# cloneofsimo/lora

Measured on AMD Instinct MI355X. Metric: train steps/sec SD1.5 rank-4 512^2 (train_lora_dreambooth.py step), higher is better.
Workload: dtype bf16

## Files before the change

### include/lora_amd.h

```cpp
#ifndef LORA_AMD_H
#define LORA_AMD_H

#include <stddef.h>
#include <stdint.h>

#ifdef __cplusplus
extern "C" {
#endif

#define LORA_AMD_ABI_VERSION 7

#define LORA_AMD_OK 0
#define LORA_AMD_EINVAL (-1)
#define LORA_AMD_ERANK (-2)
#define LORA_AMD_ELAUNCH (-3)
#define LORA_AMD_EWORKSPACE (-4)
#define LORA_AMD_EUNSUPPORTED (-5)

#define LORA_AMD_MAX_RANK 64

#define LORA_AMD_F32 0
#define LORA_AMD_F16 1
#define LORA_AMD_BF16 2

// ... 445 lines not shown
                                  int32_t r, int32_t act_dtype, float scale, float dropout_p, uint64_t seed, uint64_t offset,
                                  const uint64_t *offset_dev, void *stream);
int lora_amd_sum_parts(const float *part, int32_t nparts, int64_t stride, float *out, int64_t n, void *stream);


size_t lora_amd_sumsq_workspace(int64_t n);
int lora_amd_sumsq(const float *g, int64_t n, float *out_sumsq, void *workspace,
                   size_t workspace_bytes, void *stream);

typedef struct lora_amd_adamw_group {
  int64_t begin, end;
  float lr;
  float weight_decay;
} lora_amd_adamw_group;

int lora_amd_clip_adamw(float *p, float *g, float *exp_avg, float *exp_avg_sq,
                        int64_t n, const lora_amd_adamw_group *groups_dev,
                        int32_t n_groups, const float *sumsq, float grad_scale,
                        float max_norm, float beta1, float beta2, float eps,
                        int64_t step, int32_t zero_grad, void *stream);

int lora_amd_clip_adamw_dev(float *p, float *g, float *exp_avg, float *exp_avg_sq,
                            int64_t n, const lora_amd_adamw_group *groups_dev,
                            int32_t n_groups, const float *sumsq, float grad_scale,
                            float max_norm, float beta1, float beta2, float eps,
                            const int64_t *step_dev, const float *scaler, int32_t zero_grad, void *stream);
int lora_amd_step_advance(int64_t *step_dev, void *stream);

int lora_amd_loss_scale_update(float *state, const float *sumsq, int64_t *step_dev, float growth_factor,
                               float backoff_factor, int32_t growth_interval, void *stream);

int lora_amd_ti_rows_step(void *table, const void *table_grad, const int64_t *ids_dev, int32_t n_tokens,
                          int32_t hidden, int32_t table_dtype, float *rows, float *exp_avg, float *exp_avg_sq,
                          float lr, float beta1, float beta2, float eps, float weight_decay, float grad_scale,
                          int64_t step, float decay_lambda, float target_norm, void *stream);


size_t lora_amd_groupnorm_workspace(int32_t B, int32_t C, int32_t HW, int32_t groups);
int lora_amd_groupnorm_supported(int32_t B, int32_t C, int32_t HW, int32_t groups);
int lora_amd_groupnorm_fwd(const void *x, const void *gamma, const void *beta, void *y, float *stats,
                           void *workspace, size_t workspace_bytes, int32_t B, int32_t C, int32_t HW,
                           int32_t groups, float eps, int32_t act, int32_t dtype, void *stream);
int lora_amd_groupnorm_bwd(const void *x, const void *gout, const void *gamma, const void *beta,
                           const float *stats, void *dx, void *workspace, size_t workspace_bytes, int32_t B,
                           int32_t C, int32_t HW, int32_t groups, int32_t act, int32_t dtype, void *stream);

size_t lora_amd_groupnorm_nhwc_workspace(int32_t B, int32_t C, int32_t HW, int32_t groups);
int lora_amd_groupnorm_nhwc_fwd(const void *x, const void *gamma, const void *beta, const float *addend, void *y,
                                float *aff, void *workspace, size_t workspace_bytes, int32_t B, int32_t C, int32_t HW,
                                int32_t groups, float eps, int32_t act, int32_t dtype, void *stream);
int lora_amd_groupnorm_nhwc_bwd(const void *x, const void *gout, const void *gamma, const float *aff, void *dx,
                                void *workspace, size_t workspace_bytes, int32_t B, int32_t C, int32_t HW,
                                int32_t groups, int32_t act, int32_t dtype, void *stream);

int lora_amd_layernorm_supported(int32_t K);
int lora_amd_layernorm_fwd(const void *x, const void *gamma, const void *beta, void *y, float *stats, int64_t M,
                           int32_t K, float eps, int32_t dtype, void *stream);
int lora_amd_layernorm_bwd(const void *x, const void *gout, const void *gamma, const float *stats, void *dx,
                           int64_t M, int32_t K, int32_t dtype, void *stream);
int lora_amd_add_layernorm_fwd(const void *x, const void *res, const void *gamma, const void *beta, void *sum_out,
                               void *y, float *stats, int64_t M, int32_t K, float eps, int32_t dtype, void *stream);
int lora_amd_add_layernorm_bwd(const void *x, const void *gout, const void *gsum, const void *gamma,
                               const float *stats, void *dx, int64_t M, int32_t K, int32_t dtype, void *stream);

int lora_amd_geglu_fwd(const void *y, int64_t ldy, void *out, int64_t ldo, int64_t M, int32_t inner, int32_t dtype,
                       void *stream);
int lora_amd_geglu_bwd(const void *y, int64_t ldy, const void *gout, int64_t ldg, void *gy, int64_t ldgy, int64_t M,
                       int32_t inner, int32_t dtype, void *stream);

#ifdef __cplusplus
}
#endif
#endif
```

### lora_amd/_C.py

```python
from __future__ import annotations

import ctypes as C
import os
from typing import Dict, Optional, Sequence, Tuple

import torch

_HERE = os.path.dirname(os.path.abspath(__file__))
LIB_PATH = os.path.join(_HERE, "csrc", "liblora_amd.so")

OK = 0
F32, F16, BF16 = 0, 1, 2
FACTOR_RK, FACTOR_KR = 0, 1
ROUND_REFERENCE, ROUND_ONCE, ROUND_DITHER = 0, 1, 2
MAX_RANK = 64
ABI_VERSION = 7

_DT = {torch.float32: F32, torch.float16: F16, torch.bfloat16: BF16}

SYMBOLS = (
    "lora_amd_abi_version", "lora_amd_last_error", "lora_amd_target_arch",
    "lora_amd_merge_plan", "lora_amd_merge_batched", "lora_amd_merge_set_tuning", "lora_amd_merge_step_set_tuning", "lora_amd_rank16_mfma", "lora_amd_factors_mfma_set_tuning",
    "lora_amd_merge_step_plan", "lora_amd_merge_step",
    "lora_amd_rowdot", "lora_amd_rowdot_masked", "lora_amd_rank_update",
    "lora_amd_colreduce_workspace", "lora_amd_colreduce",
    "lora_amd_rowdot_batched", "lora_amd_colreduce_batched", "lora_amd_chol_inverse_batched",
    "lora_amd_ragged_plan", "lora_amd_rowdot_ragged", "lora_amd_colreduce_ragged", "lora_amd_sub_ragged",
    "lora_amd_rowdot16_planes_plan", "lora_amd_rowdot16_planes", "lora_amd_rowdot16_planes_packed", "lora_amd_thin_pack",
    "lora_amd_split16_ragged", "lora_amd_split16_transpose",
    "lora_amd_split16_residual", "lora_amd_thin_gram", "lora_amd_thin_apply", "lora_amd_thin_rotate", "lora_amd_thin_select", "lora_amd_thin_clamp",
    "lora_amd_linear_plan", "lora_amd_linear_fwd", "lora_amd_linear_bwd_g", "lora_amd_linear_bwd_x",
    "lora_amd_linear_bwd_factors", "lora_amd_linear_bwd_factors_drop", "lora_amd_linear_bwd_factors_heads",
    "lora_amd_linear_factors_self_plan", "lora_amd_linear_factors_self_plan_rows", "lora_amd_linear_bwd_factors_self",
    "lora_amd_linear_factors_self_ragged_plan", "lora_amd_linear_bwd_factors_self_ragged",
    "lora_amd_factors_mfma_plan", "lora_amd_factor_pack_plan", "lora_amd_factor_pack",
    "lora_amd_factors_mfma_ragged_plan", "lora_amd_linear_bwd_factors_mfma_ragged", "lora_amd_factors_mfma_block_map",
    "lora_amd_linear_bwd_factors_mfma_ragged_mapped",
    "lora_amd_linear_gemm_fwd_heads",
    "lora_amd_reduce_batched", "lora_amd_linear_gemm_supported", "lora_amd_linear_gemm_fwd",
    "lora_amd_ws_config", "lora_amd_ws_packed_elems", "lora_amd_ws_pack", "lora_amd_linear_ws", "lora_amd_linear_ws_heads",
    "lora_amd_conv_plan", "lora_amd_conv_down_fwd", "lora_amd_conv_up_fwd", "lora_amd_conv_bwd_g", "lora_amd_conv_bwd_x",
    "lora_amd_conv3_nhwc_plan", "lora_amd_conv3_nhwc_pack", "lora_amd_conv3_nhwc_down_fwd", "lora_amd_conv3_nhwc_bwd_dx",
    "lora_amd_conv3_nhwc_bwd_down", "lora_amd_sum_parts",
    "lora_amd_conv3_nhwc_pack_plan", "lora_amd_conv3_nhwc_pack_batched", "lora_amd_conv3_nhwc_fwd_fused",
    "lora_amd_linear_bwd_g_blocks", "lora_amd_linear_bwd_g_folded",
    "lora_amd_sumsq_workspace", "lora_amd_sumsq", "lora_amd_clip_adamw", "lora_amd_clip_adamw_dev",
    "lora_amd_step_advance", "lora_amd_loss_scale_update", "lora_amd_ti_rows_step",
    "lora_amd_groupnorm_workspace", "lora_amd_groupnorm_supported", "lora_amd_groupnorm_fwd", "lora_amd_groupnorm_bwd",
    "lora_amd_geglu_fwd", "lora_amd_geglu_bwd",
    "lora_amd_layernorm_supported", "lora_amd_layernorm_fwd", "lora_amd_layernorm_bwd",
    "lora_amd_groupnorm_nhwc_workspace", "lora_amd_groupnorm_nhwc_fwd", "lora_amd_groupnorm_nhwc_bwd",
    "lora_amd_add_layernorm_fwd", "lora_amd_add_layernorm_bwd",
    "lora_amd_linear_gemm_fwd_rowscale", "lora_amd_rank_update_rowscale", "lora_amd_conv_up_fwd_rowscale",
)


class HipExtensionMissing(RuntimeError):
    pass


class FactorsSelfPlan(C.Structure):
    _fields_ = [("supported", C.c_int32), ("rank_tile", C.c_int32), ("nparts", C.c_int32), ("reserved", C.c_int32),
                ("up_part_floats", C.c_int64), ("down_part_floats", C.c_int64)]


class SelfSite(C.Structure):
    _fields_ = [
        ("g", C.c_void_p), ("x", C.c_void_p), ("down", C.c_void_p), ("up", C.c_void_p),
        ("up_part", C.c_void_p), ("down_part", C.c_void_p),
        ("ldg", C.c_int64), ("ldx", C.c_int64), ("M", C.c_int64),
        ("N", C.c_int32), ("K", C.c_int32), ("r", C.c_int32), ("scale", C.c_float),
        ("g_head_dim", C.c_int32), ("g_head_pad", C.c_int32), ("x_head_dim", C.c_int32), ("x_head_pad", C.c_int32),
        ("rows_per_block", C.c_int32), ("nsplit", C.c_int32), ("kt_g", C.c_int32), ("logL_g", C.c_int32),
        ("kt_x", C.c_int32), ("logL_x", C.c_int32), ("tile_g", C.c_int32), ("nct_g", C.c_int32),
        ("tile_x", C.c_int32), ("nct_x", C.c_int32),
        ("reserved0", C.c_int32), ("reserved", C.c_int32),
        ("block_begin", C.c_int64),
    ]


class FactorsMfmaPlan(C.Structure):
    _fields_ = [("supported", C.c_int32), ("lds_class", C.c_int32), ("rank_tile", C.c_int32),
                ("rows_per_block", C.c_int32), ("nparts", C.c_int32), ("lds_bytes", C.c_int32),
                ("blocks_per_wg", C.c_int32), ("reserved", C.c_int32),
                ("up_part_floats", C.c_int64), ("down_part_floats", C.c_int64),
                ("pack_up_elems", C.c_int64), ("pack_down_elems", C.c_int64)]


class PackSite(C.Structure):
    _fields_ = [("down", C.c_void_p), ("up", C.c_void_p), ("pk_down", C.c_void_p), ("pk_up", C.c_void_p),
                ("N", C.c_int32), ("K", C.c_int32), ("r", C.c_int32), ("reserved", C.c_int32), ("begin", C.c_int64)]


class FmSite(C.Structure):
    _fields_ = [
        ("g", C.c_void_p), ("x", C.c_void_p), ("pk_up", C.c_void_p), ("pk_down", C.c_void_p),
        ("up_part", C.c_void_p), ("down_part", C.c_void_p),
        ("ldg", C.c_int64), ("ldx", C.c_int64), ("M", C.c_int64),
        ("N", C.c_int32), ("K", C.c_int32), ("r", C.c_int32), ("scale", C.c_float),
        ("g_head_dim", C.c_int32), ("g_head_pad", C.c_int32), ("x_head_dim", C.c_int32), ("x_head_pad", C.c_int32),
        ("rows_per_block", C.c_int32), ("blocks_per_wg", C.c_int32),
        ("resident_is_x", C.c_int32), ("cw", C.c_int32), ("nchunk", C.c_int32), ("x_head_magic", C.c_int32),
        ("g_head_magic", C.c_int32), ("lds_bytes", C.c_int32),
        ("block_begin", C.c_int64),
# ... 1912 lines not shown
    _check(require().lora_amd_layernorm_bwd(x.data_ptr(), gout.data_ptr(), gamma.data_ptr(), stats.data_ptr(),
                                            dx.data_ptr(), x.numel() // K, K, dtype_code(x.dtype), _stream()),
           "lora_amd_layernorm_bwd")
    return dx


_gn_nhwc_ws_cache: Dict[Tuple[int, int, int, int], int] = {}


def groupnorm_nhwc_workspace(B: int, C_: int, HW: int, groups: int) -> int:
    key = (B, C_, HW, groups)
    n = _gn_nhwc_ws_cache.get(key)
    if n is None:
        n = _gn_nhwc_ws_cache[key] = int(require().lora_amd_groupnorm_nhwc_workspace(B, C_, HW, groups))
    return n


def groupnorm_nhwc_fwd(x: torch.Tensor, gamma: torch.Tensor, beta: torch.Tensor, groups: int, eps: float,
                       act: bool, addend: Optional[torch.Tensor] = None) -> Tuple[torch.Tensor, torch.Tensor]:
    _dev_check(x, gamma, beta, addend)
    if addend is not None and (addend.dtype != torch.float32 or not addend.is_contiguous()
                               or tuple(addend.shape) != (x.shape[0], x.shape[1])):
        raise ValueError("groupnorm_nhwc_fwd: addend must be a contiguous float32 [B, C] tensor")
    B, C_ = x.shape[0], x.shape[1]
    HW = x.numel() // (B * C_)
    nbytes = groupnorm_nhwc_workspace(B, C_, HW, groups)
    if nbytes == 0:
        raise ValueError(f"lora_amd_groupnorm_nhwc: geometry {tuple(x.shape)} / {groups} groups not supported")
    y = torch.empty_like(x)
    aff = torch.empty(B, 4, C_, dtype=torch.float32, device=x.device)
    ws = torch.empty(nbytes // 4, dtype=torch.float32, device=x.device)
    _check(require().lora_amd_groupnorm_nhwc_fwd(x.data_ptr(), gamma.data_ptr(), beta.data_ptr(), _ptr(addend),
                                                 y.data_ptr(), aff.data_ptr(), ws.data_ptr(), nbytes, B, C_, HW, groups, eps,
                                                 1 if act else 0, dtype_code(x.dtype), _stream()),
           "lora_amd_groupnorm_nhwc_fwd")
    return y, aff


def groupnorm_nhwc_bwd(x: torch.Tensor, gout: torch.Tensor, gamma: torch.Tensor, aff: torch.Tensor, groups: int,
                       act: bool) -> torch.Tensor:
    _dev_check(x, gout, gamma, aff)
    B, C_ = x.shape[0], x.shape[1]
    HW = x.numel() // (B * C_)
    nbytes = groupnorm_nhwc_workspace(B, C_, HW, groups)
    dx = torch.empty_like(x)
    ws = torch.empty(nbytes // 4, dtype=torch.float32, device=x.device)
    _check(require().lora_amd_groupnorm_nhwc_bwd(x.data_ptr(), gout.data_ptr(), gamma.data_ptr(), aff.data_ptr(),
                                                 dx.data_ptr(), ws.data_ptr(), nbytes, B, C_, HW, groups,
                                                 1 if act else 0, dtype_code(x.dtype), _stream()),
           "lora_amd_groupnorm_nhwc_bwd")
    return dx


def add_layernorm_fwd(x: torch.Tensor, res: torch.Tensor, gamma: torch.Tensor, beta: torch.Tensor,
                      eps: float) -> Tuple[torch.Tensor, torch.Tensor, torch.Tensor]:
    _dev_check(x, res, gamma, beta)
    K = x.shape[-1]
    M = x.numel() // K
    s, y = torch.empty_like(x), torch.empty_like(x)
    stats = torch.empty(M, 2, dtype=torch.float32, device=x.device)
    _check(require().lora_amd_add_layernorm_fwd(x.data_ptr(), res.data_ptr(), gamma.data_ptr(), beta.data_ptr(),
                                                s.data_ptr(), y.data_ptr(), stats.data_ptr(), M, K, eps,
                                                dtype_code(x.dtype), _stream()), "lora_amd_add_layernorm_fwd")
    return s, y, stats


def add_layernorm_bwd(s: torch.Tensor, gout: torch.Tensor, gsum: Optional[torch.Tensor], gamma: torch.Tensor,
                      stats: torch.Tensor) -> torch.Tensor:
    _dev_check(s, gout, gsum, gamma, stats)
    K = s.shape[-1]
    dx = torch.empty_like(s)
    _check(require().lora_amd_add_layernorm_bwd(s.data_ptr(), gout.data_ptr(), _ptr(gsum), gamma.data_ptr(),
                                                stats.data_ptr(), dx.data_ptr(), s.numel() // K, K,
                                                dtype_code(s.dtype), _stream()), "lora_amd_add_layernorm_bwd")
    return dx
```

### lora_amd/csrc/hostops.hip

```cpp
#include <algorithm>

#include "common.hpp"

namespace lora_amd {

constexpr int kHT = 256;
constexpr int kHU = 4;
constexpr int kHMaxSlices = 256;

__device__ inline float fast_rcp(float v) { return __builtin_amdgcn_rcpf(v); }
__device__ inline float sigmoidf(float z) { return fast_rcp(1.f + __expf(-z)); }
__device__ inline float silu_grad(float z) {
  const float s = sigmoidf(z);
  return s * (1.f + z * (1.f - s));
}
__device__ inline float erf_as(float x) {
  const float ax = fabsf(x);
  const float t = fast_rcp(1.f + 0.3275911f * ax);
  float p = 1.061405429f;
  p = fmaf(p, t, -1.453152027f);
  p = fmaf(p, t, 1.421413741f);
  p = fmaf(p, t, -0.284496736f);
  p = fmaf(p, t, 0.254829592f);
  const float e = 1.f - p * t * __expf(-ax * ax);
// ... 474 lines not shown
  const float c1 = group_allsum(s1, logL) * inv_n, c2 = group_allsum(s2, logL) * inv_n;
  if (!live) return;
#pragma unroll
  for (int u = 0; u < kLU; ++u) {
    const int cc = l + u * L;
    if (cc < c8) {
      float o[8];
#pragma unroll
      for (int e = 0; e < 8; ++e) o[e] = rstd * (t[u][e] - c1 - xh[u][e] * c2);
      if (ADDG) {
        float gs[8];
        unpack8_sel<E>(gsr[u], true, gs);
#pragma unroll
        for (int e = 0; e < 8; ++e) o[e] += gs[e];
      }
      store8<E>(dx + row * (int64_t)c8 * 8 + cc * 8, o);
    }
  }
}

static inline int ln_logL(int c8) {
  for (int lg = 0; lg <= 6; ++lg)
    if (((c8 + (1 << lg) - 1) >> lg) <= kLU) return lg;
  return -1;
}

constexpr int kNU = 4;

struct GnNhwcGeo {
  int c8, cw, tiles, nslots, px, S;
  bool ok;
};
static GnNhwcGeo gn_nhwc_geo(int B, int C, int HW, int G) {
  GnNhwcGeo q{};
  q.ok = B > 0 && C > 0 && HW > 0 && G > 0 && C % G == 0 && C % 8 == 0;
  if (!q.ok) return q;
  q.c8 = C / 8;
  int best = 1, best_act = 0;
  for (int d = 1; d <= std::min(q.c8, 128); ++d) {
    if (q.c8 % d) continue;
    const int act = (kHT / d) * d;
    if (act >= best_act) { best_act = act; best = d; }
  }
  q.cw = best;
  q.tiles = q.c8 / q.cw;
  q.nslots = kHT / q.cw;
  int64_t px = std::max<int64_t>(2 * q.nslots, (int64_t)HW * B * q.tiles / 768);
  px = std::min<int64_t>(px, HW);
  q.px = (int)px;
  q.S = (HW + q.px - 1) / q.px;
  return q;
}

struct NhwcBlock {
  int b, s, col, slot, np;
  bool active;
  int64_t base;
};
__device__ inline NhwcBlock nhwc_block(int C, int HW, int cw, int tiles, int nslots, int px, int S) {
  NhwcBlock k;
  const int bs = blockIdx.x / tiles, tile = blockIdx.x - bs * tiles;
  k.b = bs / S;
  k.s = bs - k.b * S;
  k.slot = threadIdx.x / cw;
  const int cl = threadIdx.x - k.slot * cw;
  k.active = k.slot < nslots;
  k.col = tile * cw + cl;
  const int p0 = k.s * px;
  k.np = min(px, HW - p0);
  k.base = ((int64_t)k.b * HW + p0) * C + (int64_t)k.col * 8;
  return k;
}

__device__ inline void ld8f(const float *p, float (&v)[8]) {
  typedef float f4 __attribute__((ext_vector_type(4)));
  const f4 a = *reinterpret_cast<const f4 *>(p), b = *reinterpret_cast<const f4 *>(p + 4);
#pragma unroll
  for (int i = 0; i < 4; ++i) { v[i] = a[i]; v[i + 4] = b[i]; }
}
__device__ inline void st8f(float *p, const float (&v)[8]) {
  typedef float f4 __attribute__((ext_vector_type(4)));
  f4 a, b;
#pragma unroll
  for (int i = 0; i < 4; ++i) { a[i] = v[i]; b[i] = v[i + 4]; }
  *reinterpret_cast<f4 *>(p) = a;
  *reinterpret_cast<f4 *>(p + 4) = b;
}

__device__ inline void nhwc_slot_reduce(float (&a0)[8], float (&a1)[8], const NhwcBlock &k, int cw, int nslots,
                                        float *s_red ) {
  if (k.active) {
    st8f(s_red + (size_t)threadIdx.x * 8, a0);
    st8f(s_red + (size_t)(kHT + threadIdx.x) * 8, a1);
  }
  __syncthreads();
  if (k.active && k.slot == 0) {
    for (int sl = 1; sl < nslots; ++sl) {
      float t0[8], t1[8];
      ld8f(s_red + (size_t)(sl * cw + threadIdx.x) * 8, t0);
      ld8f(s_red + (size_t)(kHT + sl * cw + threadIdx.x) * 8, t1);
#pragma unroll
      for (int e = 0; e < 8; ++e) { a0[e] += t0[e]; a1[e] += t1[e]; }
    }
  }
}

// ... 172 lines not shown
      }
      LORA_AMD_LOADS_ISSUED();
#pragma unroll
      for (int u = 0; u < kNU; ++u) {
        const int pp = p + u * nslots;
        if (pp < k.np) {
          float v[8], go[8], t[8], xh[8];
          unpack8_sel<E>(xr[u], true, v);
          unpack8_sel<E>(gr[u], true, go);
          gn_nhwc_terms<E, ACT>(v, go, ga, be, mean, rstd, gam, t, xh);
          if (APPLY) {
            float o[8];
#pragma unroll
            for (int e = 0; e < 8; ++e) o[e] = rstd[e] * (t[e] - c1[e] - xh[e] * c2[e]);
            store8<E>(dx + k.base + (int64_t)pp * C, o);
          } else {
#pragma unroll
            for (int e = 0; e < 8; ++e) {
              s1[e] += t[e];
              s2[e] = fmaf(t[e], xh[e], s2[e]);
            }
          }
        }
      }
    }
  }
  if (!APPLY) {
    nhwc_slot_reduce(s1, s2, k, cw, nslots, s_red);
    if (k.active && k.slot == 0) {
      float *o = part + ((int64_t)(k.b * S + k.s) * 2) * C + (int64_t)k.col * 8;
      st8f(o, s1);
      st8f(o + C, s2);
    }
  }
}

__global__ __launch_bounds__(kHT) void gn_nhwc_bwd_finalize_kernel(const float *__restrict__ part,
                                                                   float *__restrict__ cvec, int C, int HW, int G,
                                                                   int S) {
  __shared__ float s_red[4][2];
  const int b = blockIdx.x / G, g = blockIdx.x - b * G, cpg = C / G;
  float s1 = 0.f, s2 = 0.f;
  for (int i = threadIdx.x; i < S * cpg; i += kHT) {
    const int s = i / cpg, c = g * cpg + (i - s * cpg);
    const float *pp = part + ((int64_t)(b * S + s) * 2) * C + c;
    s1 += pp[0];
    s2 += pp[C];
  }
  block_sum2(s1, s2, s_red);
  const float inv_n = 1.f / ((float)HW * (float)cpg);
  for (int cc = threadIdx.x; cc < cpg; cc += kHT) {
    cvec[(int64_t)b * 2 * C + g * cpg + cc] = s1 * inv_n;
    cvec[(int64_t)b * 2 * C + C + g * cpg + cc] = s2 * inv_n;
  }
}

static inline bool aligned_for(const void *p, int dt) { return ((uintptr_t)p % (dt == LORA_AMD_F32 ? 32 : 16)) == 0; }

}

using namespace lora_amd;

extern "C" size_t lora_amd_groupnorm_workspace(int32_t B, int32_t C, int32_t HW, int32_t groups) {
  const GnGeo q = gn_geo(B, C, HW, groups);
  return q.ok ? (size_t)B * groups * q.S * 2 * sizeof(float) : 0;
}

extern "C" int lora_amd_groupnorm_supported(int32_t B, int32_t C, int32_t HW, int32_t groups) {
  return gn_geo(B, C, HW, groups).ok ? 1 : 0;
}

#define GN_CHECKS(name)                                                                                              \
  const GnGeo q = gn_geo(B, C, HW, groups);                                                                          \
  LORA_AMD_CHECK(q.ok, LORA_AMD_EINVAL, name ": geometry B=%d C=%d HW=%d groups=%d not supported", B, C, HW, groups); \
  LORA_AMD_CHECK(dtype_ok(dtype), LORA_AMD_EINVAL, name ": bad dtype %d", dtype);                                    \
  LORA_AMD_CHECK(workspace_bytes >= lora_amd_groupnorm_workspace(B, C, HW, groups), LORA_AMD_EWORKSPACE,             \
                 name ": workspace %zu < %zu bytes", workspace_bytes, lora_amd_groupnorm_workspace(B, C, HW, groups)); \
  const dim3 grid((unsigned)((int64_t)B * groups * q.S)), block(kHT);                                                \
  hipStream_t st = (hipStream_t)stream;                                                                              \
  float *part = reinterpret_cast<float *>(workspace)

extern "C" int lora_amd_groupnorm_fwd(const void *x, const void *gamma, const void *beta, void *y, float *stats,
                                      void *workspace, size_t workspace_bytes, int32_t B, int32_t C, int32_t HW,
                                      int32_t groups, float eps, int32_t act, int32_t dtype, void *stream) {
  GN_CHECKS("groupnorm_fwd");
  LORA_AMD_CHECK(x && gamma && beta && y && stats && workspace, LORA_AMD_EINVAL, "groupnorm_fwd: null pointer");
  LORA_AMD_CHECK(aligned_for(x, dtype) && aligned_for(y, dtype), LORA_AMD_EINVAL, "groupnorm_fwd: unaligned tensor");
  by_dtype(dtype, [&](auto e) {
    using E = decltype(e);
    using S = typename E::storage;
    hipLaunchKernelGGL((gn_stats_kernel<E>), grid, block, 0, st, (const S *)x, part, groups, q.cpg, HW, q.chunks,
                       q.per_block, q.S);
    by_bool(act != 0, [&](auto a) {
      hipLaunchKernelGGL((gn_apply_kernel<E, decltype(a)::value>), grid, block, 0, st, (const S *)x, (const S *)gamma,
                         (const S *)beta, (S *)y, part, stats, groups, q.cpg, HW, q.chunks, q.per_block, q.S, eps);
    });
  });
  return check_launch("lora_amd_groupnorm_fwd");
}

extern "C" int lora_amd_groupnorm_bwd(const void *x, const void *gout, const void *gamma, const void *beta,
                                      const float *stats, void *dx, void *workspace, size_t workspace_bytes,
                                      int32_t B, int32_t C, int32_t HW, int32_t groups, int32_t act, int32_t dtype,
                                      void *stream) {
  GN_CHECKS("groupnorm_bwd");
  LORA_AMD_CHECK(x && gout && gamma && beta && stats && dx && workspace, LORA_AMD_EINVAL,
// ... 77 lines not shown
}

extern "C" int lora_amd_add_layernorm_fwd(const void *x, const void *res, const void *gamma, const void *beta,
                                          void *sum_out, void *y, float *stats, int64_t M, int32_t K, float eps,
                                          int32_t dtype, void *stream) {
  LN_CHECKS("layernorm_fwd");
  LORA_AMD_CHECK(x && gamma && beta && y && stats, LORA_AMD_EINVAL, "layernorm_fwd: null pointer");
  LORA_AMD_CHECK((res == nullptr) == (sum_out == nullptr), LORA_AMD_EINVAL,
                 "layernorm_fwd: res and sum_out go together");
  LORA_AMD_CHECK(aligned_for(x, dtype) && aligned_for(y, dtype) && aligned_for(gamma, dtype) && aligned_for(beta, dtype) &&
                     aligned_for(res, dtype) && aligned_for(sum_out, dtype),
                 LORA_AMD_EINVAL, "layernorm_fwd: unaligned tensor");
  const bool add = res != nullptr;
  by_dtype(dtype, [&](auto e) {
    by_bool(add, [&](auto a) {
      using S = typename decltype(e)::storage;
      hipLaunchKernelGGL((ln_fwd_kernel<decltype(e), decltype(a)::value>), grid, block, 0, st, (const S *)x, (const S *)res,
                         (const S *)gamma, (const S *)beta, (S *)sum_out, (S *)y, stats, M, c8, logL, eps);
    });
  });
  return check_launch("lora_amd_layernorm_fwd");
}

extern "C" int lora_amd_layernorm_bwd(const void *x, const void *gout, const void *gamma, const float *stats,
                                      void *dx, int64_t M, int32_t K, int32_t dtype, void *stream) {
  return lora_amd_add_layernorm_bwd(x, gout, nullptr, gamma, stats, dx, M, K, dtype, stream);
}

extern "C" int lora_amd_add_layernorm_bwd(const void *x, const void *gout, const void *gsum, const void *gamma,
                                          const float *stats, void *dx, int64_t M, int32_t K, int32_t dtype,
                                          void *stream) {
  LN_CHECKS("layernorm_bwd");
  LORA_AMD_CHECK(x && gout && gamma && stats && dx, LORA_AMD_EINVAL, "layernorm_bwd: null pointer");
  LORA_AMD_CHECK(aligned_for(x, dtype) && aligned_for(gout, dtype) && aligned_for(dx, dtype) && aligned_for(gamma, dtype) &&
                     aligned_for(gsum, dtype),
                 LORA_AMD_EINVAL, "layernorm_bwd: unaligned tensor");
  by_dtype(dtype, [&](auto e) {
    by_bool(gsum != nullptr, [&](auto a) {
      using S = typename decltype(e)::storage;
      hipLaunchKernelGGL((ln_bwd_kernel<decltype(e), decltype(a)::value>), grid, block, 0, st, (const S *)x, (const S *)gout,
                         (const S *)gsum, (const S *)gamma, stats, (S *)dx, M, c8, logL);
    });
  });
  return check_launch("lora_amd_layernorm_bwd");
}

static size_t gn_nhwc_part_floats(const GnNhwcGeo &q, int B, int C) { return (size_t)B * q.S * 2 * C; }

extern "C" size_t lora_amd_groupnorm_nhwc_workspace(int32_t B, int32_t C, int32_t HW, int32_t groups) {
  const GnNhwcGeo q = gn_nhwc_geo(B, C, HW, groups);
  return q.ok ? (gn_nhwc_part_floats(q, B, C) + (size_t)B * 2 * C) * sizeof(float) : 0;
}

#define GN_NHWC_CHECKS(name)                                                                                          \
  const GnNhwcGeo q = gn_nhwc_geo(B, C, HW, groups);                                                                  \
  LORA_AMD_CHECK(q.ok, LORA_AMD_EINVAL, name ": geometry B=%d C=%d HW=%d groups=%d not supported", B, C, HW, groups); \
  LORA_AMD_CHECK(dtype_ok(dtype), LORA_AMD_EINVAL, name ": bad dtype %d", dtype);                                     \
  LORA_AMD_CHECK(workspace_bytes >= lora_amd_groupnorm_nhwc_workspace(B, C, HW, groups), LORA_AMD_EWORKSPACE,         \
                 name ": workspace %zu bytes too small", workspace_bytes);                                            \
  const dim3 grid((unsigned)((int64_t)B * q.S * q.tiles)), gridg((unsigned)(B * groups)), block(kHT);                 \
  hipStream_t st = (hipStream_t)stream;                                                                               \
  float *part = reinterpret_cast<float *>(workspace);                                                                 \
  float *cvec = part + gn_nhwc_part_floats(q, B, C);                                                                  \
  (void)cvec

extern "C" int lora_amd_groupnorm_nhwc_fwd(const void *x, const void *gamma, const void *beta, const float *addend,
                                           void *y, float *aff, void *workspace, size_t workspace_bytes, int32_t B, int32_t C, int32_t HW,
                                           int32_t groups, float eps, int32_t act, int32_t dtype, void *stream) {
  GN_NHWC_CHECKS("groupnorm_nhwc_fwd");
  LORA_AMD_CHECK(x && gamma && beta && y && aff && workspace, LORA_AMD_EINVAL, "groupnorm_nhwc_fwd: null pointer");
  LORA_AMD_CHECK(aligned_for(x, dtype) && aligned_for(y, dtype) && ((uintptr_t)aff % 32) == 0, LORA_AMD_EINVAL,
                 "groupnorm_nhwc_fwd: unaligned tensor");
  by_dtype(dtype, [&](auto e) {
    using E = decltype(e);
    using S = typename E::storage;
    hipLaunchKernelGGL((gn_nhwc_stats_kernel<E>), grid, block, 0, st, (const S *)x, part, C, HW, q.cw, q.tiles,
                       q.nslots, q.px, q.S);
    hipLaunchKernelGGL((gn_nhwc_finalize_kernel<E>), gridg, block, 0, st, part, (const S *)gamma, (const S *)beta,
                       addend, aff, C, HW, groups, q.px, q.S, eps);
    by_bool(act != 0, [&](auto a) {
      hipLaunchKernelGGL((gn_nhwc_apply_kernel<E, decltype(a)::value>), grid, block, 0, st, (const S *)x, aff, (S *)y, C, HW,
                         q.cw, q.tiles, q.nslots, q.px, q.S);
    });
  });
  return check_launch("lora_amd_groupnorm_nhwc_fwd");
}

extern "C" int lora_amd_groupnorm_nhwc_bwd(const void *x, const void *gout, const void *gamma, const float *aff,
                                           void *dx, void *workspace, size_t workspace_bytes, int32_t B, int32_t C,
                                           int32_t HW, int32_t groups, int32_t act, int32_t dtype, void *stream) {
  GN_NHWC_CHECKS("groupnorm_nhwc_bwd");
  LORA_AMD_CHECK(x && gout && gamma && aff && dx && workspace, LORA_AMD_EINVAL, "groupnorm_nhwc_bwd: null pointer");
  LORA_AMD_CHECK(aligned_for(x, dtype) && aligned_for(gout, dtype) && aligned_for(dx, dtype) &&
                     aligned_for(gamma, dtype) && ((uintptr_t)aff % 32) == 0,
                 LORA_AMD_EINVAL, "groupnorm_nhwc_bwd: unaligned tensor");
  by_dtype(dtype, [&](auto e) {
    by_bool(act != 0, [&](auto a) {
      using E = decltype(e);
      using S = typename E::storage;
      constexpr bool A = decltype(a)::value;
      hipLaunchKernelGGL((gn_nhwc_bwd_kernel<E, A, false>), grid, block, 0, st, (const S *)x, (const S *)gout,
                         (const S *)gamma, aff, part, (const float *)nullptr, (S *)nullptr, C, HW, q.cw, q.tiles,
                         q.nslots, q.px, q.S);
      hipLaunchKernelGGL(gn_nhwc_bwd_finalize_kernel, gridg, block, 0, st, part, cvec, C, HW, groups, q.S);
      hipLaunchKernelGGL((gn_nhwc_bwd_kernel<E, A, true>), grid, block, 0, st, (const S *)x, (const S *)gout,
                         (const S *)gamma, aff, (float *)nullptr, cvec, (S *)dx, C, HW, q.cw, q.tiles, q.nslots,
                         q.px, q.S);
    });
  });
  return check_launch("lora_amd_groupnorm_nhwc_bwd");
}
```

### lora_amd/ops.py

```python
from __future__ import annotations

import os

from typing import Optional

import torch
import torch.nn.functional as F

from . import _C

def next_dropout_stream(device) -> tuple:
    seed = int(torch.initial_seed()) & 0xFFFFFFFFFFFFFFFF
    pool = _POOL.get("buf")
    if pool is not None and pool.device == torch.device(device):
        i = _POOL["next"]
        if i >= pool.numel():
            pool = _POOL["buf"] = torch.empty(_POOL_SIZE, dtype=torch.int64, device=device).random_(0, 1 << 62)
            i = 0
        _POOL["next"] = i + 1
        return seed, pool[i:i + 1]
    off = torch.empty(1, dtype=torch.int64, device=device).random_(0, 1 << 62)
    return seed, off


# ... 365 lines not shown
                _C.linear_bwd_g(g2, t, up_c, gt_part, up_part, s, p, seed, off)
                dx2 = (g2 @ weight) if need_x else None
                if dx2 is not None and not _C._rows_ok(dx2):
                    dx2 = dx2.contiguous()
                _C.linear_bwd_x(x2, dx2, gt_part, plan.nct_g, down_c, sel, down_part)
            if need_x:
                dx = dx2.view(ctx.x_shape)
            if sink is not None:
                sink.pending = key
            else:
                gt_part, up_part, down_part = bufs()
                d_up = torch.empty((N, r), dtype=torch.float32, device=g2.device)
                d_down = torch.empty((r, K), dtype=torch.float32, device=g2.device)
                rows = [(up_part, d_up, plan.nparts_up, plan.rank_tile, N, r, _C.FACTOR_KR, 1.0, 0.0),
                        (down_part, d_down, plan.nparts_down, plan.rank_tile, K, r, _C.FACTOR_RK, 1.0, 0.0)]
                table, n, total = _C.make_reduce_table(rows, g2.device)
                _C.reduce_batched(table, n, total)
                d_up, d_down = d_up.to(up.dtype), d_down.to(down.dtype)
        else:
            gt = None
            _log("bwd", "primitives", M, K, N, r)
            if need_x or need_down:
                gt = rowdot_any(g2, up_c, _C.FACTOR_KR, s, sel, True, p, seed, off)
            if need_up:
                if sink is not None:
                    colreduce_any(g2, t, _C.FACTOR_KR, s, out=sink.up_grad, beta=1.0, p=p, seed=seed, off=off)
                else:
                    d_up = colreduce_any(g2, t, _C.FACTOR_KR, s, p=p, seed=seed, off=off).to(up.dtype)
            if need_down:
                if sink is not None:
                    colreduce_any(x2, gt, _C.FACTOR_RK, 1.0, out=sink.down_grad, beta=1.0)
                else:
                    d_down = colreduce_any(x2, gt, _C.FACTOR_RK, 1.0).to(down.dtype)
            if need_x:
                dx2 = g2 @ weight
                rank_update_any_(dx2, gt, down_c, _C.FACTOR_RK, 1.0)
                dx = dx2.view(ctx.x_shape)
        dw = g2.t() @ x2 if need_w else None
        db = g2.sum(0) if (ctx.has_bias and need_b) else None
        return dx, dw, db, d_down, d_up, None, None, None, None, None, None


TRANSPOSED_DX = True
DEFER_MASKED_FACTORS = True
CONCAT_GROUPS = True
RANK16_MFMA = True
FM_TWO_CLASSES = True
CONCURRENT_FACTOR_LAUNCHES = False
FM_LONGEST_FIRST = True
FM_LONGEST_FIRST_CLASS1 = False
FM_BLOCK_MAP = True
CONV3_FUSED = True
MASTER_MERGE = True


def apply_ab_overrides(spec: str, namespace: dict) -> dict:
    allowed = ("TRANSPOSED_DX", "DEFER_MASKED_FACTORS", "CONCAT_GROUPS", "RANK16_MFMA", "FM_TWO_CLASSES", "CONCURRENT_FACTOR_LAUNCHES", "FM_LONGEST_FIRST", "FM_LONGEST_FIRST_CLASS1", "FM_BLOCK_MAP", "CONV3_FUSED", "MASTER_MERGE", "WS_HEADS", "WS_DROPOUT",
               "WS_DROPOUT_WIDE",
               "WS_DROPOUT_WIDE_BWD")
    done = {}
    for item in filter(None, (s.strip() for s in spec.split(","))):
        name, _, val = item.partition("=")
        if name not in allowed:
            raise ValueError(f"LORA_AMD_AB: unknown constant {name!r} (one of {', '.join(allowed)})")
        namespace[name] = done[name] = val.strip() not in ("0", "", "false", "False")
    return done


apply_ab_overrides(os.environ.get("LORA_AMD_AB", ""), globals())
if not RANK16_MFMA and _C.available():
    _C.rank16_mfma(0)

MERGE_ROUNDING = _C.ROUND_ONCE if os.environ.get("LORA_AMD_MERGE_ROUNDING", "dither") == "once" else _C.ROUND_DITHER


def master_site(w: torch.Tensor, dt: torch.dtype) -> bool:
    return MASTER_MERGE and w.dtype == torch.float32 and dt in (torch.bfloat16, torch.float16) and not w.requires_grad


def _gemm_range():
    if PATH_LOG is not None:
        return torch.profiler.record_function("lora_amd::merged_gemm")
    import contextlib

    return contextlib.nullcontext()


class MergedWeights:

    def __init__(self, state=None):
        self.entries = {}
        self._plans = None
        self.refreshes = 0
        self._state = state
        self._fresh_at = None
        self.defer_factors = state is not None
        self._owed = []
        self._tables = {}
        self._packs = {}
        self._pack_tables = {}
        self._graph_keep = []
        self.groups = {}
        self._keys = {}

    def lookup(self, module, w, b, dt, in_heads, out_heads, need_dx: bool = True):
        e = self._entry(module, w, b, dt, in_heads, out_heads)
        if need_dx and TRANSPOSED_DX and e["w_eff_t"] is None and (e["step"] or (in_heads is None and w.shape[0] % 32 == 0)):
            self._add_transposed(e)
        return e["w_eff"], e["b_eff"], e["w_eff_t"]

    def _refresh_if_stale(self) -> None:
        if (self._state is not None and self._fresh_at != self._state.step_count
                and not torch.cuda.is_current_stream_capturing()):
            self.refresh()

    def _entry(self, module, w, b, dt, in_heads, out_heads, out=None):
        self._refresh_if_stale()
        key = (id(module), in_heads, out_heads, dt)
        e = self.entries.get(key)
        if e is not None and (e["ptrs"] != (module.lora_up.weight.data_ptr(), module.lora_down.weight.data_ptr(),
                                            w.data_ptr()) or e["scale"] != float(module.scale)):
            if e.get("group") is not None:
                self.groups.pop(e["group"], None)
            e = None
# ... 1175 lines not shown
```

Baseline: 35.86.

## Fuse NHWC GroupNorm forward and backward into single-launch register-resident kernels

Adds single-kernel NHWC GroupNorm forward and backward paths. One block covers a bundle of channels for one batch item, keeps the pixels in registers, and does the group reductions in shared memory. This replaces the earlier multi-launch pipeline (partial sums, finalize, apply) when the per-thread pixel count fits a small register budget. The aim is to cut launch overhead and to avoid re-reading activations and writing a workspace. In exchange it adds register pressure, may lower occupancy from few blocks per group, and relies on a template dispatch over capacities. It is on by default and can be turned off through an A/B override.

```diff
diff --git a/include/lora_amd.h b/include/lora_amd.h
--- a/include/lora_amd.h
+++ b/include/lora_amd.h
@@ -521,6 +521,8 @@
 int lora_amd_groupnorm_nhwc_bwd(const void *x, const void *gout, const void *gamma, const float *aff, void *dx,
                                 void *workspace, size_t workspace_bytes, int32_t B, int32_t C, int32_t HW,
                                 int32_t groups, int32_t act, int32_t dtype, void *stream);
+int lora_amd_groupnorm_nhwc_launches(int32_t B, int32_t C, int32_t HW, int32_t groups, int32_t dtype);
+int lora_amd_groupnorm_nhwc_set_tuning(int32_t one_launch);
 
 int lora_amd_layernorm_supported(int32_t K);
 int lora_amd_layernorm_fwd(const void *x, const void *gamma, const void *beta, void *y, float *stats, int64_t M,
diff --git a/lora_amd/_C.py b/lora_amd/_C.py
--- a/lora_amd/_C.py
+++ b/lora_amd/_C.py
@@ -50,6 +50,7 @@
     "lora_amd_geglu_fwd", "lora_amd_geglu_bwd",
     "lora_amd_layernorm_supported", "lora_amd_layernorm_fwd", "lora_amd_layernorm_bwd",
     "lora_amd_groupnorm_nhwc_workspace", "lora_amd_groupnorm_nhwc_fwd", "lora_amd_groupnorm_nhwc_bwd",
+    "lora_amd_groupnorm_nhwc_launches", "lora_amd_groupnorm_nhwc_set_tuning",
     "lora_amd_add_layernorm_fwd", "lora_amd_add_layernorm_bwd",
     "lora_amd_linear_gemm_fwd_rowscale", "lora_amd_rank_update_rowscale", "lora_amd_conv_up_fwd_rowscale",
 )
@@ -2068,6 +2069,20 @@
     return dx
 
 
+def groupnorm_nhwc_launches(B: int, C_: int, HW: int, groups: int, dtype: torch.dtype) -> int:
+    lib = require()
+    lib.lora_amd_groupnorm_nhwc_launches.argtypes = [C.c_int32] * 5
+    lib.lora_amd_groupnorm_nhwc_launches.restype = C.c_int
+    return int(lib.lora_amd_groupnorm_nhwc_launches(B, C_, HW, groups, dtype_code(dtype)))
+
+
+def groupnorm_nhwc_set_tuning(one_launch: int = -1) -> int:
+    lib = require()
+    lib.lora_amd_groupnorm_nhwc_set_tuning.argtypes = [C.c_int32]
+    lib.lora_amd_groupnorm_nhwc_set_tuning.restype = C.c_int
+    return int(lib.lora_amd_groupnorm_nhwc_set_tuning(int(one_launch)))
+
+
 def add_layernorm_fwd(x: torch.Tensor, res: torch.Tensor, gamma: torch.Tensor, beta: torch.Tensor,
                       eps: float) -> Tuple[torch.Tensor, torch.Tensor, torch.Tensor]:
     _dev_check(x, res, gamma, beta)
diff --git a/lora_amd/csrc/hostops.hip b/lora_amd/csrc/hostops.hip
--- a/lora_amd/csrc/hostops.hip
+++ b/lora_amd/csrc/hostops.hip
@@ -550,6 +550,34 @@
   return q;
 }
 
+constexpr int kGnOneMaxChunks = 32;
+constexpr int kGnOneMaxBytes = 256;
+static int g_gn_one_launch = 1;
+
+struct GnOneGeo {
+  int cpg, bundle, nslots, ppt;
+  bool ok;
+};
+static GnOneGeo gn_one_geo(int C, int HW, int G) {
+  GnOneGeo o{};
+  o.cpg = C / G;
+  int g8 = 8;
+  while (o.cpg % g8) g8 >>= 1;
+  const int64_t bundle = (int64_t)o.cpg * (8 / g8);
+  if (bundle > kGnOneMaxChunks * 8 || (int64_t)HW * C > INT32_MAX) return o;
+  o.bundle = (int)bundle;
+  o.nslots = kHT / (o.bundle / 8);
+  o.ppt = (HW + o.nslots - 1) / o.nslots;
+  o.ok = true;
+  return o;
+}
+static int gn_nhwc_route(int B, int C, int HW, int G, int dtype) {
+  if (!gn_nhwc_geo(B, C, HW, G).ok || !dtype_ok(dtype)) return 0;
+  if (!g_gn_one_launch) return 3;
+  const GnOneGeo o = gn_one_geo(C, HW, G);
+  return o.ok && (int64_t)o.ppt * 8 * dtype_size(dtype) <= kGnOneMaxBytes ? 1 : 3;
+}
+
 struct NhwcBlock {
   int b, s, col, slot, np;
   bool active;
@@ -828,6 +856,233 @@
   for (int cc = threadIdx.x; cc < cpg; cc += kHT) {
     cvec[(int64_t)b * 2 * C + g * cpg + cc] = s1 * inv_n;
     cvec[(int64_t)b * 2 * C + C + g * cpg + cc] = s2 * inv_n;
+  }
+}
+
+struct GnOneBlock {
+  int slot, cl;
+  bool active;
+  int64_t base;
+  int64_t cb;
+  int gi[8];
+};
+__device__ inline GnOneBlock gn_one_block(int C, int HW, int cpg, int bundle, int nslots) {
+  GnOneBlock k;
+  const int bc8 = bundle / 8, nb = C / bundle;
+  const int b = blockIdx.x / nb, bun = blockIdx.x - b * nb;
+  k.slot = threadIdx.x / bc8;
+  k.cl = threadIdx.x - k.slot * bc8;
+  k.active = k.slot < nslots;
+  k.cb = (int64_t)bun * bundle + k.cl * 8;
+  k.base = (int64_t)b * HW * C + k.cb;
+  int g = (k.cl * 8) / cpg, r = k.cl * 8 - g * cpg;
+#pragma unroll
+  for (int e = 0; e < 8; ++e) {
+    k.gi[e] = g;
+    if (++r == cpg) { r = 0; ++g; }
+  }
+  return k;
+}
+
+template <class E, int P>
+__device__ inline void gn_one_keep_raw(Raw8<E> (&r)[P]) {
+#pragma unroll
+  for (int u = 0; u < P; ++u) asm volatile("" : "+v"(r[u].v));
+}
+
+template <int N>
+__device__ inline void gn_one_group_sums(const float (&v)[N][8], float (&tot)[N][8], const GnOneBlock &k, int cpg,
+                                         int bundle, int nsl , float *s_part, float *s_ch,
+                                         float *s_g) {
+  const int tid = threadIdx.x;
+  if (k.slot < nsl) {
+#pragma unroll
+    for (int n = 0; n < N; ++n) st8f(s_part + n * kHT * 8 + k.slot * bundle + k.cl * 8, v[n]);
+  }
+  __syncthreads();
+  if (tid < bundle) {
+#pragma unroll
+    for (int n = 0; n < N; ++n) {
+      float a = 0.f;
+      for (int sl = 0; sl < nsl; ++sl) a += s_part[n * kHT * 8 + sl * bundle + tid];
+      s_ch[n * kGnOneMaxChunks * 8 + tid] = a;
+    }
+  }
+  __syncthreads();
+  const int g = tid >> 5, l = tid & 31;
+  const bool live = g * cpg < bundle;
+#pragma unroll
+  for (int n = 0; n < N; ++n) {
+    float a = 0.f;
+    if (live)
+      for (int j = l; j < cpg; j += 32) a += s_ch[n * kGnOneMaxChunks * 8 + g * cpg + j];
+#pragma unroll
+    for (int off = 16; off > 0; off >>= 1) a += __shfl_xor(a, off, 64);
+    if (live && l == 0) s_g[n * 8 + g] = a;
+  }
+  __syncthreads();
+#pragma unroll
+  for (int n = 0; n < N; ++n)
+#pragma unroll
+    for (int e = 0; e < 8; ++e) tot[n][e] = s_g[n * 8 + k.gi[e]];
+}
+
+template <class E, bool ACT, int P>
+__global__ __launch_bounds__(kHT) void gn_nhwc_one_fwd_kernel(const typename E::storage *__restrict__ x,
+                                                              const typename E::storage *__restrict__ gamma,
+                                                              const typename E::storage *__restrict__ beta,
+                                                              const float *__restrict__ addend,
+                                                              typename E::storage *__restrict__ y,
+                                                              float *__restrict__ aff, int C, int HW, int cpg,
+                                                              int bundle, int nslots, float eps) {
+  __shared__ __attribute__((aligned(16))) float s_part[kHT * 8];
+  __shared__ float s_ch[kGnOneMaxChunks * 8], s_g[8];
+  const GnOneBlock k = gn_one_block(C, HW, cpg, bundle, nslots);
+  const int b = blockIdx.x / (C / bundle);
+  Raw8<E> xr[P];
+#pragma unroll
+  for (int u = 0; u < P; ++u) {
+    const int pp = k.slot + u * nslots;
+    xr[u] = load8_raw<E>(x + k.base + (k.active && pp < HW ? pp : 0) * C);
+  }
+  const Raw8<E> gr = load8_raw<E>(gamma + k.cb), br = load8_raw<E>(beta + k.cb);
+  float add[8];
+  ld8f_sel(addend != nullptr ? addend + (int64_t)b * C + k.cb : aff, addend != nullptr, add);
+  LORA_AMD_LOADS_ISSUED();
+  float s[1][8], tot[1][8], m[8];
+  int cnt = 0;
+#pragma unroll
+  for (int e = 0; e < 8; ++e) s[0][e] = 0.f;
+#pragma unroll
+  for (int u = 0; u < P; ++u) {
+    const bool ok = k.active && k.slot + u * nslots < HW;
+    float v[8];
+    unpack8_sel<E>(xr[u], ok, v);
+    cnt += ok ? 1 : 0;
+#pragma unroll
+    for (int e = 0; e < 8; ++e) s[0][e] += v[e];
+  }
+#pragma unroll
+  for (int e = 0; e < 8; ++e) s[0][e] = fmaf((float)cnt, add[e], s[0][e]);
+  const int nsl = min(nslots, HW);
+  const float inv_n = 1.f / ((float)HW * (float)cpg);
+  gn_one_group_sums<1>(s, tot, k, cpg, bundle, nsl, s_part, s_ch, s_g);
+#pragma unroll
+  for (int e = 0; e < 8; ++e) {
+    m[e] = tot[0][e] * inv_n - add[e];
+    s[0][e] = 0.f;
+  }
+  gn_one_keep_raw(xr);
+#pragma unroll
+  for (int u = 0; u < P; ++u) {
+    const bool ok = k.active && k.slot + u * nslots < HW;
+    float v[8];
+    unpack8_sel<E>(xr[u], true, v);
+#pragma unroll
+    for (int e = 0; e < 8; ++e) {
+      const float d = ok ? v[e] - m[e] : 0.f;
+      s[0][e] = fmaf(d, d, s[0][e]);
+    }
+  }
+  gn_one_group_sums<1>(s, tot, k, cpg, bundle, nsl, s_part, s_ch, s_g);
+  gn_one_keep_raw(xr);
+  float ga[8], be[8], rstd[8];
+  unpack8_sel<E>(gr, true, ga);
+  unpack8_sel<E>(br, true, be);
+#pragma unroll
+  for (int e = 0; e < 8; ++e) {
+    rstd[e] = rsqrtf(tot[0][e] * inv_n + eps);
+    ga[e] *= rstd[e];
+    be[e] = fmaf(-m[e], ga[e], be[e]);
+  }
+  if (k.slot == 0) {
+    float *o = aff + (int64_t)b * 4 * C + k.cb;
+    st8f(o, ga);
+    st8f(o + C, be);
+    st8f(o + 2 * C, m);
+    st8f(o + 3 * C, rstd);
+  }
+#pragma unroll
+  for (int u = 0; u < P; ++u) {
+    const int pp = k.slot + u * nslots;
+    if (k.active && pp < HW) {
+      float v[8], o[8];
+      unpack8_sel<E>(xr[u], true, v);
+#pragma unroll
+      for (int e = 0; e < 8; ++e) {
+        const float z = fmaf(v[e], ga[e], be[e]);
+        o[e] = ACT ? z * sigmoidf(z) : z;
+      }
+      store8<E>(y + k.base + pp * C, o);
+    }
+  }
+}
+
+template <class E, bool ACT, int P>
+__global__ __launch_bounds__(kHT) void gn_nhwc_one_bwd_kernel(const typename E::storage *__restrict__ x,
+                                                              const typename E::storage *__restrict__ gout,
+                                                              const typename E::storage *__restrict__ gamma,
+                                                              const float *__restrict__ aff,
+                                                              typename E::storage *__restrict__ dx, int C, int HW,
+                                                              int cpg, int bundle, int nslots) {
+  __shared__ __attribute__((aligned(16))) float s_part[2 * kHT * 8];
+  __shared__ float s_ch[2 * kGnOneMaxChunks * 8], s_g[2 * 8];
+  const GnOneBlock k = gn_one_block(C, HW, cpg, bundle, nslots);
+  const int b = blockIdx.x / (C / bundle);
+  Raw8<E> xr[P], gr[P];
+  const auto off = [&](int u) {
+    const int pp = k.slot + u * nslots;
+    return k.base + (k.active && pp < HW ? pp : 0) * C;
+  };
+#pragma unroll
+  for (int u = 0; u < P; ++u) xr[u] = load8_raw<E>(x + off(u));
+#pragma unroll
+  for (int u = 0; u < P; ++u) gr[u] = load8_raw<E>(gout + off(u));
+  float ga[8], be[8], mean[8], rstd[8], gam[8];
+  const float *ab = aff + (int64_t)b * 4 * C + k.cb;
+  ld8f_sel(ab, true, ga);
+  ld8f_sel(ab + C, true, be);
+  ld8f_sel(ab + 2 * C, true, mean);
+  ld8f_sel(ab + 3 * C, true, rstd);
+  unpack8_sel<E>(load8_raw<E>(gamma + k.cb), true, gam);
+  LORA_AMD_LOADS_ISSUED();
+  float s[2][8], tot[2][8];
+#pragma unroll
+  for (int e = 0; e < 8; ++e) s[0][e] = s[1][e] = 0.f;
+#pragma unroll
+  for (int u = 0; u < P; ++u) {
+    const bool ok = k.active && k.slot + u * nslots < HW;
+    float v[8], go[8], t[8], xh[8];
+    unpack8_sel<E>(xr[u], true, v);
+    unpack8_sel<E>(gr[u], ok, go);
+    gn_nhwc_terms<E, ACT>(v, go, ga, be, mean, rstd, gam, t, xh);
+#pragma unroll
+    for (int e = 0; e < 8; ++e) {
+      s[0][e] += t[e];
+      s[1][e] = fmaf(t[e], xh[e], s[1][e]);
+    }
+  }
+  gn_one_group_sums<2>(s, tot, k, cpg, bundle, min(nslots, HW), s_part, s_ch, s_g);
+  gn_one_keep_raw(xr);
+  gn_one_keep_raw(gr);
+  const float inv_n = 1.f / ((float)HW * (float)cpg);
+  float c1[8], c2[8];
+#pragma unroll
+  for (int e = 0; e < 8; ++e) {
+    c1[e] = tot[0][e] * inv_n;
+    c2[e] = tot[1][e] * inv_n;
+  }
+#pragma unroll
+  for (int u = 0; u < P; ++u) {
+    if (k.active && k.slot + u * nslots < HW) {
+      float v[8], go[8], t[8], xh[8], o[8];
+      unpack8_sel<E>(xr[u], true, v);
+      unpack8_sel<E>(gr[u], true, go);
+      gn_nhwc_terms<E, ACT>(v, go, ga, be, mean, rstd, gam, t, xh);
+#pragma unroll
+      for (int e = 0; e < 8; ++e) o[e] = rstd[e] * (t[e] - c1[e] - xh[e] * c2[e]);
+      store8<E>(dx + off(u), o);
+    }
   }
 }
 
@@ -1011,6 +1266,36 @@
   return q.ok ? (gn_nhwc_part_floats(q, B, C) + (size_t)B * 2 * C) * sizeof(float) : 0;
 }
 
+extern "C" int lora_amd_groupnorm_nhwc_launches(int32_t B, int32_t C, int32_t HW, int32_t groups, int32_t dtype) {
+  return gn_nhwc_route(B, C, HW, groups, dtype);
+}
+
+extern "C" int lora_amd_groupnorm_nhwc_set_tuning(int32_t one_launch) {
+  const int prev = g_gn_one_launch;
+  if (one_launch == 0 || one_launch == 1) g_gn_one_launch = one_launch;
+  return prev;
+}
+
+template <int V, int... Vs, class F>
+static inline auto by_capacity(int v, F &&f) {
+  if constexpr (sizeof...(Vs) == 0) {
+    return f(int_c<V>);
+  } else {
+    if (v <= V) return f(int_c<V>);
+    return by_capacity<Vs...>(v, f);
+  }
+}
+template <class E, class F>
+static inline auto gn_one_by_pixels(int ppt, F &&f) {
+  if constexpr (sizeof(typename E::storage) == 4) {
+    static_assert(8 * 32 == kGnOneMaxBytes, "largest f32 capacity");
+    return by_capacity<2, 4, 8>(ppt, f);
+  } else {
+    static_assert(16 * 16 == kGnOneMaxBytes, "largest 16-bit capacity");
+    return by_capacity<2, 4, 8, 16>(ppt, f);
+  }
+}
+
 #define GN_NHWC_CHECKS(name)                                                                                          \
   const GnNhwcGeo q = gn_nhwc_geo(B, C, HW, groups);                                                                  \
   LORA_AMD_CHECK(q.ok, LORA_AMD_EINVAL, name ": geometry B=%d C=%d HW=%d groups=%d not supported", B, C, HW, groups); \
@@ -1030,6 +1315,23 @@
   LORA_AMD_CHECK(x && gamma && beta && y && aff && workspace, LORA_AMD_EINVAL, "groupnorm_nhwc_fwd: null pointer");
   LORA_AMD_CHECK(aligned_for(x, dtype) && aligned_for(y, dtype) && ((uintptr_t)aff % 32) == 0, LORA_AMD_EINVAL,
                  "groupnorm_nhwc_fwd: unaligned tensor");
+  if (gn_nhwc_route(B, C, HW, groups, dtype) == 1 && aligned_for(gamma, dtype) && aligned_for(beta, dtype) &&
+      ((uintptr_t)addend % 16) == 0) {
+    const GnOneGeo o = gn_one_geo(C, HW, groups);
+    const dim3 grid1((unsigned)((int64_t)B * (C / o.bundle)));
+    by_dtype(dtype, [&](auto e) {
+      by_bool(act != 0, [&](auto a) {
+        gn_one_by_pixels<decltype(e)>(o.ppt, [&](auto p) {
+          using E = decltype(e);
+          using S = typename E::storage;
+          hipLaunchKernelGGL((gn_nhwc_one_fwd_kernel<E, decltype(a)::value, decltype(p)::value>), grid1, block, 0, st,
+                             (const S *)x, (const S *)gamma, (const S *)beta, addend, (S *)y, aff, C, HW, o.cpg, o.bundle,
+                             o.nslots, eps);
+        });
+      });
+    });
+    return check_launch("lora_amd_groupnorm_nhwc_fwd");
+  }
   by_dtype(dtype, [&](auto e) {
     using E = decltype(e);
     using S = typename E::storage;
@@ -1053,6 +1355,22 @@
   LORA_AMD_CHECK(aligned_for(x, dtype) && aligned_for(gout, dtype) && aligned_for(dx, dtype) &&
                      aligned_for(gamma, dtype) && ((uintptr_t)aff % 32) == 0,
                  LORA_AMD_EINVAL, "groupnorm_nhwc_bwd: unaligned tensor");
+  if (gn_nhwc_route(B, C, HW, groups, dtype) == 1) {
+    const GnOneGeo o = gn_one_geo(C, HW, groups);
+    const dim3 grid1((unsigned)((int64_t)B * (C / o.bundle)));
+    by_dtype(dtype, [&](auto e) {
+      by_bool(act != 0, [&](auto a) {
+        gn_one_by_pixels<decltype(e)>(o.ppt, [&](auto p) {
+          using E = decltype(e);
+          using S = typename E::storage;
+          hipLaunchKernelGGL((gn_nhwc_one_bwd_kernel<E, decltype(a)::value, decltype(p)::value>), grid1, block, 0, st,
+                             (const S *)x, (const S *)gout, (const S *)gamma, aff, (S *)dx, C, HW, o.cpg, o.bundle,
+                             o.nslots);
+        });
+      });
+    });
+    return check_launch("lora_amd_groupnorm_nhwc_bwd");
+  }
   by_dtype(dtype, [&](auto e) {
     by_bool(act != 0, [&](auto a) {
       using E = decltype(e);
diff --git a/lora_amd/ops.py b/lora_amd/ops.py
--- a/lora_amd/ops.py
+++ b/lora_amd/ops.py
@@ -441,10 +441,11 @@
 FM_BLOCK_MAP = True
 CONV3_FUSED = True
 MASTER_MERGE = True
+GN_ONE_LAUNCH = True
 
 
 def apply_ab_overrides(spec: str, namespace: dict) -> dict:
-    allowed = ("TRANSPOSED_DX", "DEFER_MASKED_FACTORS", "CONCAT_GROUPS", "RANK16_MFMA", "FM_TWO_CLASSES", "CONCURRENT_FACTOR_LAUNCHES", "FM_LONGEST_FIRST", "FM_LONGEST_FIRST_CLASS1", "FM_BLOCK_MAP", "CONV3_FUSED", "MASTER_MERGE", "WS_HEADS", "WS_DROPOUT",
+    allowed = ("TRANSPOSED_DX", "DEFER_MASKED_FACTORS", "CONCAT_GROUPS", "RANK16_MFMA", "FM_TWO_CLASSES", "CONCURRENT_FACTOR_LAUNCHES", "FM_LONGEST_FIRST", "FM_LONGEST_FIRST_CLASS1", "FM_BLOCK_MAP", "CONV3_FUSED", "MASTER_MERGE", "GN_ONE_LAUNCH", "WS_HEADS", "WS_DROPOUT",
                "WS_DROPOUT_WIDE",
                "WS_DROPOUT_WIDE_BWD")
     done = {}
@@ -459,6 +460,8 @@
 apply_ab_overrides(os.environ.get("LORA_AMD_AB", ""), globals())
 if not RANK16_MFMA and _C.available():
     _C.rank16_mfma(0)
+if not GN_ONE_LAUNCH and _C.available():
+    _C.groupnorm_nhwc_set_tuning(0)
 
 MERGE_ROUNDING = _C.ROUND_ONCE if os.environ.get("LORA_AMD_MERGE_ROUNDING", "dither") == "once" else _C.ROUND_DITHER
 
```

Result: no change. 36.17, median of 6 (+0.9%).
